# zyt334/AdaFace

Measured on AMD Instinct MI355X. Metric: 512x512 images/sec @ 50 DDIM steps, batch 8, higher is better.
Workload: dtype bf16

## Files before the change

### adaface_amd/csrc/af_conv_s8.hip

```cpp
#include "af_kernels.h"

#include <type_traits>

namespace cs8 {
typedef bf16 T;
typedef __attribute__((ext_vector_type(4))) unsigned u32x4;
constexpr int BM = 256, BN = 80, NI = 5, MI = 2, SPLITK = 4;
constexpr int HSLOTS = 448, HBUF = HSLOTS * 128, NHQ = HSLOTS / 8 / 8;
constexpr int WBYTES = BN * 128, WPIECES = BN / 8, D = 3, NS = 4;
constexpr int W_BASE = 2 * HBUF, LDS_BYTES = W_BASE + NS * WBYTES;
static_assert(LDS_BYTES <= 160 * 1024 && NHQ == 7, "LDS plan");

__device__ __forceinline__ void lds_dma16(__amdgpu_buffer_rsrc_t rs, char* lds_base, unsigned voffset, unsigned soffset) {
#if defined(__HIP_DEVICE_COMPILE__)
  __builtin_amdgcn_raw_ptr_buffer_load_lds(rs, (__attribute__((address_space(3))) void*)lds_base, 16, voffset, soffset, 0, 0);
#endif
}
__device__ __forceinline__ u32x4 lds_read128(unsigned addr) {
  u32x4 v;
  asm volatile("ds_read_b128 %0, %1" : "=v"(v) : "v"(addr) : "memory");
  return v;
}
template <int OFF> __device__ __forceinline__ u32x4 lds_read128o(unsigned addr) {
  u32x4 v;
  asm volatile("ds_read_b128 %0, %1 offset:%2" : "=v"(v) : "v"(addr), "n"(OFF) : "memory");
  return v;
}
template <int N> __device__ __forceinline__ void wait_vm() { asm volatile("s_waitcnt vmcnt(%0)" ::"n"(N) : "memory"); }
template <int N> __device__ __forceinline__ void wait_lgkm2(u32x4& a, u32x4& b) {
  asm volatile("s_waitcnt lgkmcnt(%2)" : "+v"(a), "+v"(b) : "n"(N) : "memory");
}
template <int N> __device__ __forceinline__ void wait_lgkm4(u32x4& a, u32x4& b, u32x4& c, u32x4& d) {
  asm volatile("s_waitcnt lgkmcnt(%4)" : "+v"(a), "+v"(b), "+v"(c), "+v"(d) : "n"(N) : "memory");
}
template <int I, int N, typename F> __device__ __forceinline__ void static_for(F&& f) {
  if constexpr (I < N) {
    f(std::integral_constant<int, I>{});
    static_for<I + 1, N>(f);
  }
}
__device__ __forceinline__ f32x4 mma(const u32x4& a, const u32x4& b, const f32x4& c) {
  return __builtin_amdgcn_mfma_f32_16x16x32_bf16(__builtin_bit_cast(bf16x8, a), __builtin_bit_cast(bf16x8, b), c, 0, 0, 0);
}

template <int SPLITK_T>
__global__ __launch_bounds__(512) void conv3x3_s8_kernel(const ConvGemmParams p) {
  extern __shared__ __attribute__((aligned(1024))) char smem[];
  const int tid = threadIdx.x, lane = tid & 63, wid = __builtin_amdgcn_readfirstlane(tid >> 6);
  const int l15 = lane & 15, g = lane >> 4;
  const int ntn = p.N / BN;
  const int tm = blockIdx.x / ntn, tn = blockIdx.x - tm * ntn;
  const int m0 = tm * BM, n0 = tn * BN, zk = blockIdx.z;
  const int nch = (p.Cin >> 6) / SPLITK_T, chunk0 = zk * nch;
  const __amdgpu_buffer_rsrc_t rs_x = __builtin_amdgcn_make_buffer_rsrc(const_cast<T*>(reinterpret_cast<const T*>(p.src)), 0, (int)0xFFFFFFF0u, 0x00020000);
  const __amdgpu_buffer_rsrc_t rs_w = __builtin_amdgcn_make_buffer_rsrc(const_cast<T*>(reinterpret_cast<const T*>(p.W)), 0, (int)0xFFFFFFF0u, 0x00020000);

  const int srow = lane >> 3;
  const unsigned dchunk = (unsigned)((lane & 7) ^ srow);
  const unsigned ldcb = (unsigned)p.ldc * 2u;
  const int wsh = p.wo_shift, Wo = 1 << wsh, HW = Wo + 2, hwsh = p.howo_shift;
  const int R = min(p.Ho, 256 >> wsh), HP1 = (R + 2) * HW, ipt = 256 / (R << wsh);
  const int img0 = m0 >> hwsh, y0 = (m0 & ((1 << hwsh) - 1)) >> wsh;
  unsigned h_off[NHQ];
#pragma unroll
  for (int q = 0; q < NHQ; ++q) {
    const int hp = (wid + 8 * q) * 8 + srow;
    const int img = hp / HP1, rem = hp - img * HP1, hy = rem / HW, hx = rem - hy * HW;
    const int iy = y0 + hy - 1, ix = hx - 1;
    const bool ok = img < ipt && (unsigned)iy < (unsigned)p.Ho && (unsigned)ix < (unsigned)Wo;
    h_off[q] = ok ? (unsigned)(((img0 + img) << hwsh) + (iy << wsh) + ix) * ldcb + dchunk * 16u : 0xFFFFFFFFu;
  }
  const int nwq = wid < WPIECES - 8 ? 2 : 1;
  unsigned w_off[2];
#pragma unroll
  for (int q = 0; q < 2; ++q) w_off[q] = (unsigned)((n0 + (wid + 8 * q) * 8 + srow) * p.ldw * 2) + dchunk * 16u;

  const int nsteps = nch * 9;
  auto stage_w = [&](int s, int slot) {
    const int c = s / 9, tap = s - 9 * c;
    const bool live = s < nsteps;
    const unsigned k0b = (unsigned)(tap * p.Cin + (chunk0 + c) * 64) * 2u;
    lds_dma16(rs_w, smem + W_BASE + slot * WBYTES + wid * 1024, live ? w_off[0] : 0xFFFFFFFFu, k0b);
    if (wid < WPIECES - 8) lds_dma16(rs_w, smem + W_BASE + slot * WBYTES + (wid + 8) * 1024, live ? w_off[1] : 0xFFFFFFFFu, k0b);
  };
  auto stage_h = [&](auto qc, int hbuf, int c) {
    constexpr int q = decltype(qc)::value;
    const bool live = c < nch;
    lds_dma16(rs_x, smem + hbuf * HBUF + (wid + 8 * q) * 1024, live ? h_off[q] : 0xFFFFFFFFu, (unsigned)(chunk0 + c) * 128u);
  };

  const unsigned lds0 = (unsigned)(__UINTPTR_TYPE__)((__attribute__((address_space(3))) char*)smem);
  const unsigned fch0 = (unsigned)(g ^ (lane & 7)) * 16u, fch1 = (unsigned)((g + 4) ^ (lane & 7)) * 16u;
  const unsigned w_base = (unsigned)(l15 * 128);
  int xhp[MI];
#pragma unroll
  for (int j = 0; j < MI; ++j) {
    const int t = wid * 32 + j * 16 + l15;
    const int part = t / (R << wsh), yl = (t >> wsh) - part * R;
    xhp[j] = part * HP1 + yl * HW + (t & (Wo - 1));
  }
  f32x4 acc[NI][MI];
#pragma unroll
  for (int i = 0; i < NI; ++i)
#pragma unroll
    for (int j = 0; j < MI; ++j) acc[i][j] = f32x4{0.f, 0.f, 0.f, 0.f};

  static_for<0, NHQ>([&](auto qc) { stage_h(qc, 0, 0); });
#pragma unroll
  for (int s = 0; s < D; ++s) stage_w(s, s);

  u32x4 xs[2][MI][2], wh[2][2][2];
#pragma unroll
  for (int j = 0; j < MI; ++j) xs[1][j][0] = xs[1][j][1] = u32x4{0u, 0u, 0u, 0u};
#pragma unroll
  for (int b2 = 0; b2 < 2; ++b2) wh[1][b2][0] = wh[1][b2][1] = u32x4{0u, 0u, 0u, 0u};
  int hb = 0, slot = 0;
  for (int c = 0; c < nch; ++c) {
    static_for<0, 9>([&](auto tc) {
      constexpr int tap = decltype(tc)::value;
      constexpr int cs = tap & 1, ps = cs ^ 1;
      constexpr int hyoung = tap == 0 ? 0 : (tap == 1 ? 1 : (tap == 2 ? 2 : (tap <= 7 ? 3 : 2)));
      if (nwq == 2) wait_vm<2 * (D - 1) + hyoung>(); else wait_vm<(D - 1) + hyoung>();
      __builtin_amdgcn_s_barrier();
      constexpr int ky = tap / 3, kx = tap - 3 * ky;
      const int tapoff = ky * HW + kx;
      unsigned xa[MI];
#pragma unroll
      for (int j = 0; j < MI; ++j) {
        const unsigned hp = (unsigned)(xhp[j] + tapoff);
        xa[j] = lds0 + (unsigned)(hb * HBUF) + (hp << 7) + ((((unsigned)g ^ hp) & 7u) << 4);
      }
      const unsigned wa0 = lds0 + (unsigned)(W_BASE + slot * WBYTES) + w_base + fch0;
      const unsigned wa1 = lds0 + (unsigned)(W_BASE + slot * WBYTES) + w_base + fch1;
      u32x4 wf[3][2];
#pragma unroll
      for (int j = 0; j < MI; ++j) {
        xs[cs][j][0] = lds_read128(xa[j]);
        xs[cs][j][1] = lds_read128(xa[j] ^ 64u);
      }
      wf[0][0] = lds_read128o<0 * 2048>(wa0); wf[0][1] = lds_read128o<0 * 2048>(wa1);
      wf[1][0] = lds_read128o<1 * 2048>(wa0); wf[1][1] = lds_read128o<1 * 2048>(wa1);
      wf[2][0] = lds_read128o<2 * 2048>(wa0); wf[2][1] = lds_read128o<2 * 2048>(wa1);
      __builtin_amdgcn_sched_barrier(0);
#pragma unroll
      for (int b2 = 0; b2 < 2; ++b2)
#pragma unroll
        for (int j = 0; j < MI; ++j) {
          acc[3 + b2][j] = mma(wh[ps][b2][0], xs[ps][j][0], acc[3 + b2][j]);
          acc[3 + b2][j] = mma(wh[ps][b2][1], xs[ps][j][1], acc[3 + b2][j]);
          asm volatile("" : "+v"(acc[3 + b2][j]));
        }
      __builtin_amdgcn_sched_barrier(0);
      wait_lgkm4<4>(xs[cs][0][0], xs[cs][0][1], xs[cs][1][0], xs[cs][1][1]);
      wait_lgkm2<4>(wf[0][0], wf[0][1]);
#pragma unroll
      for (int j = 0; j < MI; ++j) {
        acc[0][j] = mma(wf[0][0], xs[cs][j][0], acc[0][j]);
        acc[0][j] = mma(wf[0][1], xs[cs][j][1], acc[0][j]);
        asm volatile("" : "+v"(acc[0][j]));
      }
      wh[cs][0][0] = lds_read128o<3 * 2048>(wa0); wh[cs][0][1] = lds_read128o<3 * 2048>(wa1);
      __builtin_amdgcn_sched_barrier(0);
      wait_lgkm2<4>(wf[1][0], wf[1][1]);
#pragma unroll
      for (int j = 0; j < MI; ++j) {
        acc[1][j] = mma(wf[1][0], xs[cs][j][0], acc[1][j]);
        acc[1][j] = mma(wf[1][1], xs[cs][j][1], acc[1][j]);
        asm volatile("" : "+v"(acc[1][j]));
      }
      stage_w(c * 9 + tap + D, (slot + D) & (NS - 1));
      if constexpr (tap < NHQ) stage_h(std::integral_constant<int, tap>{}, hb ^ 1, c + 1);
      wh[cs][1][0] = lds_read128o<4 * 2048>(wa0); wh[cs][1][1] = lds_read128o<4 * 2048>(wa1);
      __builtin_amdgcn_sched_barrier(0);
      wait_lgkm2<4>(wf[2][0], wf[2][1]);
#pragma unroll
      for (int j = 0; j < MI; ++j) {
        acc[2][j] = mma(wf[2][0], xs[cs][j][0], acc[2][j]);
        acc[2][j] = mma(wf[2][1], xs[cs][j][1], acc[2][j]);
        asm volatile("" : "+v"(acc[2][j]));
      }
      __builtin_amdgcn_sched_barrier(0);
      asm volatile("s_waitcnt lgkmcnt(0)"
                   : "+v"(wh[cs][0][0]), "+v"(wh[cs][0][1]), "+v"(wh[cs][1][0]), "+v"(wh[cs][1][1])
                   :
                   : "memory");
      slot = (slot + 1) & (NS - 1);
    });
#pragma unroll
    for (int j = 0; j < MI; ++j) { xs[1][j][0] = xs[0][j][0]; xs[1][j][1] = xs[0][j][1]; }
#pragma unroll
    for (int b2 = 0; b2 < 2; ++b2) { wh[1][b2][0] = wh[0][b2][0]; wh[1][b2][1] = wh[0][b2][1]; }
    hb ^= 1;
  }
#pragma unroll
  for (int b2 = 0; b2 < 2; ++b2)
#pragma unroll
    for (int j = 0; j < MI; ++j) {
      acc[3 + b2][j] = mma(wh[1][b2][0], xs[1][j][0], acc[3 + b2][j]);
      acc[3 + b2][j] = mma(wh[1][b2][1], xs[1][j][1], acc[3 + b2][j]);
    }
  wait_vm<0>();

  if constexpr (SPLITK_T > 1) {
    float* slab = reinterpret_cast<float*>(p.ws) + (long)zk * p.M * p.N;
#pragma unroll
    for (int j = 0; j < MI; ++j) {
      const int m = m0 + wid * 32 + j * 16 + l15;
#pragma unroll
      for (int i = 0; i < NI; ++i) *reinterpret_cast<f32x4*>(slab + (long)m * p.N + n0 + i * 16 + 4 * g) = acc[i][j];
    }
  } else {
    __builtin_amdgcn_s_barrier();
    constexpr int OPITCH = BN * 2 + 16, OCH = BN / 8, NST = 32 * OCH / 64;
    char* otile = smem + wid * (32 * OPITCH);
    const T* res = reinterpret_cast<const T*>(p.residual);
    const T* rowb = reinterpret_cast<const T*>(p.rowbias);
    const int cl = 4 * g;
    float4 bvec[NI];
    Quad<T> bq[NI];
#pragma unroll
    for (int i = 0; i < NI; ++i) {
      bvec[i] = p.bias ? *reinterpret_cast<const float4*>(p.bias + n0 + i * 16 + cl) : float4{0.f, 0.f, 0.f, 0.f};
      if (rowb) bq[i].load(rowb + (long)(m0 >> p.howo_shift) * p.ldrb + n0 + i * 16 + cl);
    }
#pragma unroll
    for (int j = 0; j < MI; ++j) {
      const int m = m0 + wid * 32 + j * 16 + l15;
      Quad<T> rq[NI];
      if (res) {
#pragma unroll
        for (int i = 0; i < NI; ++i) rq[i].load(res + (long)m * p.ldr + n0 + i * 16 + cl);
      }
#pragma unroll
      for (int i = 0; i < NI; ++i) {
        const float* bp = reinterpret_cast<const float*>(&bvec[i]);
        Quad<T> o;
#pragma unroll
        for (int e = 0; e < 4; ++e) {
          float v = acc[i][j][e] + bp[e];
          if (rowb) v += to_f32<T>(bq[i].e[e]);
          if (res) v += to_f32<T>(rq[i].e[e]);
          o.e[e] = from_f32<T>(v);
        }
        o.store(reinterpret_cast<T*>(otile + (j * 16 + l15) * OPITCH) + i * 16 + cl);
      }
    }
    const __amdgpu_buffer_rsrc_t rs_o = __builtin_amdgcn_make_buffer_rsrc(reinterpret_cast<T*>(p.out), 0, (int)0xFFFFFFF0u, 0x00020000);
    u32x4 chunk[NST];
    unsigned orow[NST];
#pragma unroll
    for (int i = 0; i < NST; ++i) {
      const unsigned c = (unsigned)(lane + 64 * i), row = c / OCH, ch = c - row * OCH;
      orow[i] = (unsigned)(m0 + wid * 32 + (int)row) * (unsigned)(p.ldo * 2) + ch * 16u;
      chunk[i] = *reinterpret_cast<const u32x4*>(otile + row * OPITCH + ch * 16);
    }
    __builtin_amdgcn_sched_barrier(0);
#pragma unroll
    for (int i = 0; i < NST; ++i) __builtin_amdgcn_raw_buffer_store_b128(chunk[i], rs_o, orow[i], n0 * 2, 0);
    __builtin_amdgcn_sched_barrier(0);
  }
}
}

int af_conv_s8_slices(const ConvGemmParams& p, int batch) {
  auto pow2 = [](int v) { return v > 0 && (v & (v - 1)) == 0; };
  if (batch != 1 || p.fp8 || p.ks != 3 || p.stride != 1 || p.pad != 1 || p.up != 0 || p.Hi != p.Ho || p.Wi != p.Wo ||
      p.Hs != p.Ho || p.Ws != p.Wo || !pow2(p.Wo) || !pow2(p.Ho) || p.Wo < 8 || p.Wo > 64 || p.M <= 0 || p.M % cs8::BM != 0 || p.N % cs8::BN != 0 ||
      p.K != 9 * p.Cin || p.ldc < p.Cin || p.ldc % 8 != 0 || p.epilogue != AF_EPI_NONE || p.ln_stats || p.ln_stats_out || p.gn_ab || p.phase4 ||
      p.src_batch_stride != (long)p.Ho * p.Wo * p.ldc)
    return 0;
  const int R = p.Ho < 256 / p.Wo ? p.Ho : 256 / p.Wo;
  if (256 % (R * p.Wo) != 0 || (256 / (R * p.Wo)) * (R + 2) * (p.Wo + 2) > cs8::HSLOTS || (p.Ho * p.Wo > 256 && p.Ho % R != 0)) return 0;
  if (p.Wo == 8 && p.Ho == 8) return p.Cin % (64 * cs8::SPLITK) == 0 ? cs8::SPLITK : 0;
  return (p.Cin % 64 == 0 && p.ldo % 8 == 0 && (!p.residual || p.ldr % 4 == 0) && (!p.rowbias || p.ldrb % 4 == 0) && ((__UINTPTR_TYPE__)p.out & 15) == 0 &&
          (long)(p.M / cs8::BM) * (p.N / cs8::BN) >= 128) ? 1 : 0;
}
int af_launch_conv_s8(const ConvGemmParams& p, hipStream_t stream) {
  static unsigned long long attr_done4 = 0, attr_done1 = 0;
  const int sl = af_conv_s8_slices(p, 1);
  if (sl == 0 || p.splitk != sl || (sl > 1 && !p.ws) || p.wo_shift < 3 || p.howo_shift < p.wo_shift) {
    af_set_error_msg("conv_s8: shape / slice count %d not taken by the small-map kernel", p.splitk);
    return -1;
  }
  const dim3 grid((p.M / cs8::BM) * (p.N / cs8::BN), 1, sl);
  if (sl > 1) {
    if (int rc = af_ensure_dynamic_lds(attr_done4, reinterpret_cast<const void*>(&cs8::conv3x3_s8_kernel<cs8::SPLITK>), cs8::LDS_BYTES)) return rc;
    hipLaunchKernelGGL(cs8::conv3x3_s8_kernel<cs8::SPLITK>, grid, dim3(512), cs8::LDS_BYTES, stream, p);
  } else {
    if (int rc = af_ensure_dynamic_lds(attr_done1, reinterpret_cast<const void*>(&cs8::conv3x3_s8_kernel<1>), cs8::LDS_BYTES)) return rc;
    hipLaunchKernelGGL(cs8::conv3x3_s8_kernel<1>, grid, dim3(512), cs8::LDS_BYTES, stream, p);
  }
  HIP_CHECK_RET(hipGetLastError());
  return 0;
}
```

### adaface_amd/csrc/af_conv_gemm_pp_body.h

```cpp
  static_assert(SCHED == 0 || SCHED == 2, "schedules: 0 phased, 2 merged");
  constexpr bool MG = SCHED == 2;
  constexpr bool FT = GATHER && MG;
  static_assert(MG || !FP8, "fp8 operands exist on the merged schedule only");
  using C = PpCfg<BN>;
  typedef bf16 T;
  static_assert(!FP8 || LNMODE == 0, "fp8 operands: plain epilogue only");
  constexpr unsigned XE = FP8 ? 1u : 2u;
  constexpr int NI = C::NI, MI = C::MI, SLOT = C::SLOT, XBYTES = C::XBYTES;
  constexpr int XP0 = MG ? C::XP / 2 : C::XP0;
  constexpr int NX0 = XP0 / 4, NX1 = (C::XP - XP0) / 4;
  constexpr int WP0 = MG ? (C::WP / 8) * 4 : 0;
  constexpr int NW0 = WP0 / 4, NW1 = (C::WP - WP0) / 4;
  constexpr int NP0 = NX0 + NW0, NP1 = NX1 + NW1, NPMAX = NP0 > NP1 ? NP0 : NP1;
  constexpr int NXM = NX0 > NX1 ? NX0 : NX1, NWM = NW0 > NW1 ? NW0 : NW1;
  static_assert(XP0 % 4 == 0 && WP0 % 4 == 0 && NW1 >= 1, "piece split");
  extern __shared__ __attribute__((aligned(1024))) char smem[];

  const int tid = threadIdx.x, lane = tid & 63, wid = __builtin_amdgcn_readfirstlane(tid >> 6);
  const int g = wid >> 2, wq = wid & 3;
  const int ntm = (p.M + 255) / 256, ntn = p.N / BN;
  int tm, tn;
  tile_coords(blockIdx.x, gridDim.x, ntm, ntn, p.group_m, tm, tn);
  const int m0 = tm * 256, n0 = tn * BN;
  const int zk = blockIdx.z;
// ... 166 lines not shown

  const unsigned lds0 = (unsigned)(__UINTPTR_TYPE__)((__attribute__((address_space(3))) char*)smem);
  const unsigned fch0 = (unsigned)((lane >> 4) ^ (lane & 7)) * 16u;
  const unsigned fch1 = (unsigned)(((lane >> 4) + 4) ^ (lane & 7)) * 16u;
  const unsigned x_base = (unsigned)((wq * 64 + (lane & 15)) * 128);
  const unsigned w_base = (unsigned)(XBYTES + (g * C::HN + (lane & 15)) * 128);

  f32x4 acc[NI][MI];
#pragma unroll
  for (int i = 0; i < NI; ++i)
#pragma unroll
    for (int j = 0; j < MI; ++j) acc[i][j] = f32x4{0.f, 0.f, 0.f, 0.f};
  pp_u32x4 xf[MI][2], wf[NI][2];
#pragma unroll
  for (int i = 0; i < NI; ++i) wf[i][1] = pp_u32x4{0u, 0u, 0u, 0u};
#pragma unroll
  for (int j = 0; j < MI; ++j) xf[j][1] = pp_u32x4{0u, 0u, 0u, 0u};

  auto half = [&](int slot_off, auto rc, auto mc) {
    constexpr int ur = decltype(rc)::value, um = decltype(mc)::value;
    const unsigned b = lds0 + (unsigned)slot_off + (ur ? fch1 : fch0);
    pp_static_for<0, NI * MI>([&](auto nc) {
      constexpr int n = decltype(nc)::value;
      constexpr int i = n / MI, j = n % MI;
      if constexpr (n < NI) wf[n][ur] = pp_lds_read128<n * 2048>(b + w_base);
      else if constexpr (n < NI + MI) xf[n - NI][ur] = pp_lds_read128<(n - NI) * 2048>(b + x_base);
      acc[i][j] = __builtin_amdgcn_mfma_f32_16x16x32_bf16(__builtin_bit_cast(bf16x8, wf[i][um]),
                                                          __builtin_bit_cast(bf16x8, xf[j][um]), acc[i][j], 0, 0, 0);
      if constexpr (n < NI + MI) __builtin_amdgcn_sched_barrier(0);
    });
  };
  std::integral_constant<int, 0> U0;
  std::integral_constant<int, 1> U1;

  const int cl = 4 * (lane >> 4);
  float4 bias_r[NI];
  auto load_bias = [&]() {
#pragma unroll
    for (int i = 0; i < NI; ++i) {
      bias_r[i] = float4{0.f, 0.f, 0.f, 0.f};
      if (p.bias && p.splitk <= 1) bias_r[i] = *reinterpret_cast<const float4*>(p.bias + n0 + g * C::HN + i * 16 + cl);
    }
  };
  if constexpr (!MG) load_bias();

  float4 ln_cs[LNMODE == 1 ? NI : 1];
  float ln_mu[LNMODE == 1 ? MI : 1], ln_rs[LNMODE == 1 ? MI : 1];
  if constexpr (LNMODE == 1) {
#pragma unroll
    for (int i = 0; i < NI; ++i) ln_cs[i] = *reinterpret_cast<const float4*>(p.ln_colsum + n0 + g * C::HN + i * 16 + cl);
#pragma unroll
    for (int j = 0; j < MI; ++j) {
      const int m = m0 + wq * 64 + j * 16 + (lane & 15);
      float2 st = float2{0.f, 0.f};
      if (m < p.M) st = *reinterpret_cast<const float2*>(p.ln_stats + (long)m * 2);
      ln_mu[j] = st.x;
      ln_rs[j] = st.y;
    }
  }

  pp_u32x4 w8[MG ? NI : 1][2], xa8[MG ? MI : 1][2], xb8[MG ? MI : 1][2];
  int wsc8[FP8 ? NI : 1];
  int xsc8 = p.x_scale_e8;
  if constexpr (MG && !FP8) {
#pragma unroll
    for (int i = 0; i < NI; ++i) w8[i][0] = w8[i][1] = pp_u32x4{0u, 0u, 0u, 0u};
#pragma unroll
    for (int j = 0; j < MI; ++j) xa8[j][0] = xa8[j][1] = xb8[j][0] = xb8[j][1] = pp_u32x4{0u, 0u, 0u, 0u};
  }
  if constexpr (FP8) {
    asm volatile("" : "+v"(xsc8));
#pragma unroll
    for (int i = 0; i < NI; ++i) {
      w8[i][0] = w8[i][1] = pp_u32x4{0u, 0u, 0u, 0u};
      wsc8[i] = (int)p.w_scale[n0 + g * C::HN + i * 16 + (lane & 15)];
    }
#pragma unroll
    for (int j = 0; j < MI; ++j) xa8[j][0] = xa8[j][1] = xb8[j][0] = xb8[j][1] = pp_u32x4{0u, 0u, 0u, 0u};
  }
  auto mfma8 = [&](f32x4& c, const pp_u32x4 (&wv)[2], const pp_u32x4 (&xv)[2], int wscale) {
    if constexpr (!FP8) {
      c = __builtin_amdgcn_mfma_f32_16x16x32_bf16(__builtin_bit_cast(bf16x8, wv[0]), __builtin_bit_cast(bf16x8, xv[0]), c, 0, 0, 0);
      c = __builtin_amdgcn_mfma_f32_16x16x32_bf16(__builtin_bit_cast(bf16x8, wv[1]), __builtin_bit_cast(bf16x8, xv[1]), c, 0, 0, 0);
      asm volatile("" : "+v"(c));
      return;
    }
    const pp_i32x8 a = __builtin_shufflevector(__builtin_bit_cast(pp_i32x4, wv[0]), __builtin_bit_cast(pp_i32x4, wv[1]), 0, 1, 2, 3, 4, 5, 6, 7);
    const pp_i32x8 b = __builtin_shufflevector(__builtin_bit_cast(pp_i32x4, xv[0]), __builtin_bit_cast(pp_i32x4, xv[1]), 0, 1, 2, 3, 4, 5, 6, 7);
    c = __builtin_amdgcn_mfma_scale_f32_16x16x128_f8f6f4(a, b, c, 0, 0, 0, wscale, 0, xsc8);
    asm volatile("" : "+v"(c));
  };
  auto wait_block = [&](auto nc, pp_u32x4 (&blk)[2]) {
    constexpr int n = decltype(nc)::value;
    asm volatile("s_waitcnt lgkmcnt(%2)" : "+v"(blk[0]), "+v"(blk[1]) : "n"(n) : "memory");
  };
#ifdef AF_LAB_ABLATE
  const int lab = p.ablate >> 4;
#else
  constexpr int lab = 0;
#endif
  auto cphase8 = [&](int slot_off, pp_u32x4 (&xc)[MG ? MI : 1][2], pp_u32x4 (&xp)[MG ? MI : 1][2], int stage_off,
                     const StageCtx& sc) {
    if constexpr (MG) {
      constexpr int NB = NI + MI;
      char* sbase = smem + stage_off;
      const unsigned b0 = lds0 + (unsigned)slot_off + fch0, b1 = lds0 + (unsigned)slot_off + fch1;
      auto rd_block = [&](auto bc) {
        constexpr int bi = decltype(bc)::value;
        if (lab & 2) return;
        if constexpr (bi == 0) {
          w8[0][0] = pp_lds_read128<0>(b0 + w_base);
          w8[0][1] = pp_lds_read128<0>(b1 + w_base);
        } else if constexpr (bi <= MI) {
          xc[bi - 1][0] = pp_lds_read128<(bi - 1) * 2048>(b0 + x_base);
          xc[bi - 1][1] = pp_lds_read128<(bi - 1) * 2048>(b1 + x_base);
        } else {
          w8[bi - MI][0] = pp_lds_read128<(bi - MI) * 2048>(b0 + w_base);
          w8[bi - MI][1] = pp_lds_read128<(bi - MI) * 2048>(b1 + w_base);
        }
      };
      rd_block(std::integral_constant<int, 0>{});
      rd_block(std::integral_constant<int, 1>{});
      __builtin_amdgcn_sched_barrier(0);
      pp_static_for<0, MI * NI>([&](auto mc) {
        constexpr int m = decltype(mc)::value;
        if constexpr (m < MI) {
          if (!(lab & 4)) mfma8(acc[NI - 1][m], w8[NI - 1], xp[m], wsc8[FP8 ? NI - 1 : 0]);
        } else {
          constexpr int i = (m - MI) / MI, j = (m - MI) % MI;
          constexpr int issued = (2 + m) < NB ? (2 + m) : NB;
          constexpr int need = i == 0 ? 1 + j : (j == 0 ? MI + i : -1);
          if constexpr (need >= 0) {
            std::integral_constant<int, 2 * (issued - need - 1)> cnt;
            if constexpr (i == 0) wait_block(cnt, xc[j]); else wait_block(cnt, w8[i]);
            if constexpr (i == 0 && j == 0) wait_block(cnt, w8[0]);
          }
          if (!(lab & 4)) mfma8(acc[i][j], w8[i], xc[j], wsc8[FP8 ? i : 0]);
        }
        if constexpr (2 + m < NB) rd_block(std::integral_constant<int, 2 + m>{});
        if constexpr (m >= MI && (m - MI) / 2 < NPMAX) {
          if (!(lab & 1) && g == ((m - MI) & 1)) stage_piece(std::integral_constant<int, (m - MI) / 2>{}, sbase, sc);
        }
        __builtin_amdgcn_sched_barrier(0);
      });
      static_assert(MI + 2 * (NPMAX - 1) + 1 < MI * NI, "merged schedule: a staging slot behind an MFMA for every piece");
      pp_wait_lgkm0();
    }
  };

  int rd = 0, w0 = SLOT, w1 = 2 * SLOT;
  if constexpr (MG) {
    stage(0);
    stage(SLOT);
    auto tile = [&](auto& xc, auto& xp) {
      if (g == 0) pp_wait_vm<NP0>(); else pp_wait_vm<NP1>();
      __builtin_amdgcn_s_barrier();
      const StageCtx sc = stage_begin(kw);
      cphase8(rd, xc, xp, w1, sc);
      kw = kw_next(kw);
      const int tmp = rd; rd = w0; w0 = w1; w1 = tmp;
    };
    for (int t = 0; t + 1 < KT; t += 2) {
      tile(xa8, xb8);
      tile(xb8, xa8);
    }
    if (KT & 1) tile(xa8, xb8);
    pp_wait_vm<0>();
    if (KT & 1) {
#pragma unroll
      for (int j = 0; j < MI; ++j) mfma8(acc[NI - 1][j], w8[NI - 1], xa8[j], wsc8[FP8 ? NI - 1 : 0]);
    } else {
#pragma unroll
      for (int j = 0; j < MI; ++j) mfma8(acc[NI - 1][j], w8[NI - 1], xb8[j], wsc8[FP8 ? NI - 1 : 0]);
    }
    __builtin_amdgcn_s_barrier();
  } else {
    auto wait_keep1 = [&]() { if (g == 0) pp_wait_vm<NP0>(); else pp_wait_vm<NP1>(); };
    stage(0);
    if (g == 1) {
      if (KT > 1) { stage(SLOT); wait_keep1(); } else pp_wait_vm<0>();
    }
    __builtin_amdgcn_s_barrier();
    if (g == 1) __builtin_amdgcn_s_barrier();
    auto dphase = [&](int t) {
      if (g == 0) {
        if (t + 1 < KT) { stage(w0); wait_keep1(); } else pp_wait_vm<0>();
      } else {
        if (t + 2 < KT) stage(w1);
      }
      __builtin_amdgcn_s_barrier();
    };
    auto cend = [&](int t) {
      if (g == 1) { if (t + 2 < KT) wait_keep1(); else pp_wait_vm<0>(); }
      __builtin_amdgcn_s_barrier();
      const int tmp = rd; rd = w0; w0 = w1; w1 = tmp;
    };
    for (int t = 0; t < KT; ++t) {
      dphase(t);
      __builtin_amdgcn_s_setprio(1);
      half(rd, U0, U1);
      pp_wait_lgkm0();
      half(rd, U1, U0);
      pp_wait_lgkm0();
      __builtin_amdgcn_s_setprio(0);
      cend(t);
    }
#pragma unroll
    for (int i = 0; i < NI; ++i)
#pragma unroll
      for (int j = 0; j < MI; ++j)
        acc[i][j] = __builtin_amdgcn_mfma_f32_16x16x32_bf16(__builtin_bit_cast(bf16x8, wf[i][1]),
                                                            __builtin_bit_cast(bf16x8, xf[j][1]), acc[i][j], 0, 0, 0);
    if (g == 0) __builtin_amdgcn_s_barrier();
  }
  if constexpr (MG) load_bias();
```

Before: 10.95.

## Rework small-map 3x3 conv to 4 waves with 64-row warp tiles and deeper pipelining

Result: no change. 10.99 (median of 6 runs) (+0.4%).

```diff
diff --git a/adaface_amd/csrc/af_conv_s8.hip b/adaface_amd/csrc/af_conv_s8.hip
--- a/adaface_amd/csrc/af_conv_s8.hip
+++ b/adaface_amd/csrc/af_conv_s8.hip
@@ -5,11 +5,13 @@
 namespace cs8 {
 typedef bf16 T;
 typedef __attribute__((ext_vector_type(4))) unsigned u32x4;
-constexpr int BM = 256, BN = 80, NI = 5, MI = 2, SPLITK = 4;
-constexpr int HSLOTS = 448, HBUF = HSLOTS * 128, NHQ = HSLOTS / 8 / 8;
+constexpr int BM = 256, BN = 80, NI = 5, SPLITK = 4;
+constexpr int MI = 4, NHQ = 448 / 8 / 4;
+constexpr int MI8 = 2;
+constexpr int HSLOTS = 448, HBUF = HSLOTS * 128, NHQ8 = HSLOTS / 8 / 8;
 constexpr int WBYTES = BN * 128, WPIECES = BN / 8, D = 3, NS = 4;
 constexpr int W_BASE = 2 * HBUF, LDS_BYTES = W_BASE + NS * WBYTES;
-static_assert(LDS_BYTES <= 160 * 1024 && NHQ == 7, "LDS plan");
+static_assert(LDS_BYTES <= 160 * 1024 && NHQ8 == 7 && NHQ == 14 && NS == 4, "LDS plan");
 
 __device__ __forceinline__ void lds_dma16(__amdgpu_buffer_rsrc_t rs, char* lds_base, unsigned voffset, unsigned soffset) {
 #if defined(__HIP_DEVICE_COMPILE__)
@@ -43,8 +45,16 @@
   return __builtin_amdgcn_mfma_f32_16x16x32_bf16(__builtin_bit_cast(bf16x8, a), __builtin_bit_cast(bf16x8, b), c, 0, 0, 0);
 }
 
+template <int N> __device__ __forceinline__ void wait_lgkm_xw(u32x4 (&x)[MI][2], u32x4 (&w)[3][2]) {
+  asm volatile("s_waitcnt lgkmcnt(%14)"
+               : "+v"(x[0][0]), "+v"(x[0][1]), "+v"(x[1][0]), "+v"(x[1][1]), "+v"(x[2][0]), "+v"(x[2][1]), "+v"(x[3][0]), "+v"(x[3][1]),
+                 "+v"(w[0][0]), "+v"(w[0][1]), "+v"(w[1][0]), "+v"(w[1][1]), "+v"(w[2][0]), "+v"(w[2][1])
+               : "n"(N)
+               : "memory");
+}
+
 template <int SPLITK_T>
-__global__ __launch_bounds__(512) void conv3x3_s8_kernel(const ConvGemmParams p) {
+__global__ __launch_bounds__(256) void conv3x3_s8_kernel(const ConvGemmParams p) {
   extern __shared__ __attribute__((aligned(1024))) char smem[];
   const int tid = threadIdx.x, lane = tid & 63, wid = __builtin_amdgcn_readfirstlane(tid >> 6);
   const int l15 = lane & 15, g = lane >> 4;
@@ -61,9 +71,245 @@
   const int wsh = p.wo_shift, Wo = 1 << wsh, HW = Wo + 2, hwsh = p.howo_shift;
   const int R = min(p.Ho, 256 >> wsh), HP1 = (R + 2) * HW, ipt = 256 / (R << wsh);
   const int img0 = m0 >> hwsh, y0 = (m0 & ((1 << hwsh) - 1)) >> wsh;
+  const unsigned mg_hp1 = (1u << 18) / (unsigned)HP1 + 1u, mg_hw = (1u << 18) / (unsigned)HW + 1u;
   unsigned h_off[NHQ];
 #pragma unroll
   for (int q = 0; q < NHQ; ++q) {
+    const int hp = (wid + 4 * q) * 8 + srow;
+    const int img = (int)(((unsigned)hp * mg_hp1) >> 18), rem = hp - img * HP1, hy = (int)(((unsigned)rem * mg_hw) >> 18), hx = rem - hy * HW;
+    const int iy = y0 + hy - 1, ix = hx - 1;
+    const bool ok = img < ipt && (unsigned)iy < (unsigned)p.Ho && (unsigned)ix < (unsigned)Wo;
+    h_off[q] = ok ? (unsigned)(((img0 + img) << hwsh) + (iy << wsh) + ix) * ldcb + dchunk * 16u : 0xFFFFFFFFu;
+  }
+  const int nw = wid < WPIECES - 8 ? 3 : 2;
+  unsigned w_off[3];
+#pragma unroll
+  for (int q = 0; q < 3; ++q) w_off[q] = (unsigned)((n0 + (wid + 4 * q) * 8 + srow) * p.ldw * 2) + dchunk * 16u;
+
+  auto stage_w = [&](auto qc, int c, int tap, int slot) {
+    constexpr int q = decltype(qc)::value;
+    const unsigned k0b = (unsigned)(tap * p.Cin + (chunk0 + c) * 64) * 2u;
+    lds_dma16(rs_w, smem + W_BASE + slot * WBYTES + (wid + 4 * q) * 1024, c < nch ? w_off[q] : 0xFFFFFFFFu, k0b);
+  };
+  auto stage_h = [&](auto qc, int hbuf, int c) {
+    constexpr int q = decltype(qc)::value;
+    lds_dma16(rs_x, smem + hbuf * HBUF + (wid + 4 * q) * 1024, c < nch ? h_off[q] : 0xFFFFFFFFu, (unsigned)(chunk0 + c) * 128u);
+  };
+
+  const unsigned lds0 = (unsigned)(__UINTPTR_TYPE__)((__attribute__((address_space(3))) char*)smem);
+  const unsigned fch0 = (unsigned)(g ^ (lane & 7)) * 16u, fch1 = (unsigned)((g + 4) ^ (lane & 7)) * 16u;
+  const unsigned w_base = (unsigned)(l15 * 128);
+  int xhp[MI];
+#pragma unroll
+  for (int j = 0; j < MI; ++j) {
+    const int t = wid * 64 + j * 16 + l15;
+    const int part = t >> min(hwsh, 8), yl = (t >> wsh) - part * R;
+    xhp[j] = part * HP1 + yl * HW + (t & (Wo - 1));
+  }
+  f32x4 acc[NI][MI];
+#pragma unroll
+  for (int i = 0; i < NI; ++i)
+#pragma unroll
+    for (int j = 0; j < MI; ++j) acc[i][j] = f32x4{0.f, 0.f, 0.f, 0.f};
+
+  u32x4 xs[2][MI][2], wf[2][3][2], wr[2][2];
+  auto xaddr = [&](int j, int hbuf, int tapoff) {
+    const unsigned hp = (unsigned)(xhp[j] + tapoff);
+    return lds0 + (unsigned)(hbuf * HBUF) + (hp << 7) + ((((unsigned)g ^ hp) & 7u) << 4);
+  };
+
+  static_for<0, NHQ>([&](auto qc) { stage_h(qc, 0, 0); });
+#pragma unroll
+  for (int s = 0; s < NS; ++s) {
+    stage_w(std::integral_constant<int, 0>{}, 0, s, s);
+    stage_w(std::integral_constant<int, 1>{}, 0, s, s);
+    if (nw == 3) stage_w(std::integral_constant<int, 2>{}, 0, s, s);
+  }
+  if (nw == 3) wait_vm<3 * 3>(); else wait_vm<3 * 2>();
+  __builtin_amdgcn_s_barrier();
+#pragma unroll
+  for (int j = 0; j < MI; ++j) {
+    const unsigned xa = xaddr(j, 0, 0);
+    xs[0][j][0] = lds_read128(xa);
+    xs[0][j][1] = lds_read128(xa ^ 64u);
+  }
+  wf[0][0][0] = lds_read128o<0 * 2048>(lds0 + (unsigned)W_BASE + w_base + fch0); wf[0][0][1] = lds_read128o<0 * 2048>(lds0 + (unsigned)W_BASE + w_base + fch1);
+  wf[0][1][0] = lds_read128o<1 * 2048>(lds0 + (unsigned)W_BASE + w_base + fch0); wf[0][1][1] = lds_read128o<1 * 2048>(lds0 + (unsigned)W_BASE + w_base + fch1);
+  wf[0][2][0] = lds_read128o<2 * 2048>(lds0 + (unsigned)W_BASE + w_base + fch0); wf[0][2][1] = lds_read128o<2 * 2048>(lds0 + (unsigned)W_BASE + w_base + fch1);
+
+  auto blk = [&](auto ic, u32x4 (&x)[MI][2], u32x4& wa, u32x4& wb, auto&& f) {
+    constexpr int i = decltype(ic)::value;
+    acc[i][0] = mma(wa, x[0][0], acc[i][0]);
+    acc[i][1] = mma(wa, x[1][0], acc[i][1]);
+    f(std::integral_constant<int, 0>{});
+    __builtin_amdgcn_sched_barrier(0);
+    acc[i][2] = mma(wa, x[2][0], acc[i][2]);
+    acc[i][3] = mma(wa, x[3][0], acc[i][3]);
+    f(std::integral_constant<int, 1>{});
+    __builtin_amdgcn_sched_barrier(0);
+    acc[i][0] = mma(wb, x[0][1], acc[i][0]);
+    acc[i][1] = mma(wb, x[1][1], acc[i][1]);
+    f(std::integral_constant<int, 2>{});
+    __builtin_amdgcn_sched_barrier(0);
+    acc[i][2] = mma(wb, x[2][1], acc[i][2]);
+    acc[i][3] = mma(wb, x[3][1], acc[i][3]);
+    f(std::integral_constant<int, 3>{});
+    asm volatile("" : "+v"(acc[i][0]), "+v"(acc[i][1]), "+v"(acc[i][2]), "+v"(acc[i][3]));
+    __builtin_amdgcn_sched_barrier(0);
+  };
+  int hb = 0, slot = 0;
+  auto chunk_body = [&](auto parc, int c) {
+    constexpr int PAR = decltype(parc)::value;
+    static_for<0, 9>([&](auto tc) {
+      constexpr int tap = decltype(tc)::value;
+      constexpr int cs = (tap + PAR) & 1, ns = cs ^ 1;
+      constexpr int tap1 = (tap + 1) % 9, ky1 = tap1 / 3, kx1 = tap1 - 3 * ky1;
+      const unsigned wsl = lds0 + (unsigned)(W_BASE + slot * WBYTES) + w_base;
+      const unsigned wa0 = wsl + fch0, wa1 = wsl + fch1;
+      wait_lgkm_xw<0>(xs[cs], wf[cs]);
+      blk(std::integral_constant<int, 0>{}, xs[cs], wf[cs][0][0], wf[cs][0][1], [&](auto kc) {
+        constexpr int k = decltype(kc)::value;
+        if constexpr (k < 2) {
+          wr[k][0] = lds_read128o<(k + 3) * 2048>(wa0);
+          wr[k][1] = lds_read128o<(k + 3) * 2048>(wa1);
+        }
+      });
+      blk(std::integral_constant<int, 1>{}, xs[cs], wf[cs][1][0], wf[cs][1][1], [](auto) {});
+      wait_lgkm4<0>(wr[0][0], wr[0][1], wr[1][0], wr[1][1]);
+      constexpr int hyoung = (tap == 0 || tap == 8) ? 0 : (tap == 1 ? 2 : 4);
+      if (nw == 3) wait_vm<2 * 3 + hyoung>(); else wait_vm<2 * 2 + hyoung>();
+      __builtin_amdgcn_s_barrier();
+      const int hb1 = tap == 8 ? hb ^ 1 : hb;
+      const int tapoff1 = ky1 * HW + kx1;
+      unsigned xa[MI];
+#pragma unroll
+      for (int j = 0; j < MI; ++j) xa[j] = xaddr(j, hb1, tapoff1);
+      const unsigned wsl1 = lds0 + (unsigned)(W_BASE + ((slot + 1) & (NS - 1)) * WBYTES) + w_base;
+      const unsigned wn0 = wsl1 + fch0, wn1 = wsl1 + fch1;
+      __builtin_amdgcn_sched_barrier(0);
+      blk(std::integral_constant<int, 2>{}, xs[cs], wf[cs][2][0], wf[cs][2][1], [&](auto kc) {
+        constexpr int k = decltype(kc)::value;
+        xs[ns][k][0] = lds_read128(xa[k]);
+        xs[ns][k][1] = lds_read128(xa[k] ^ 64u);
+      });
+      blk(std::integral_constant<int, 3>{}, xs[cs], wr[0][0], wr[0][1], [&](auto kc) {
+        constexpr int k = decltype(kc)::value;
+        if constexpr (k < 3) {
+          wf[ns][k][0] = lds_read128o<k * 2048>(wn0);
+          wf[ns][k][1] = lds_read128o<k * 2048>(wn1);
+        }
+      });
+      constexpr int tap4 = (tap + NS) % 9;
+      const int c4 = tap + NS < 9 ? c : c + 1;
+      blk(std::integral_constant<int, 4>{}, xs[cs], wr[1][0], wr[1][1], [&](auto kc) {
+        constexpr int k = decltype(kc)::value;
+        if constexpr (k == 0) {
+          if constexpr (2 * tap + 1 < NHQ) {
+            stage_h(std::integral_constant<int, 2 * tap>{}, hb ^ 1, c + 1);
+            stage_h(std::integral_constant<int, 2 * tap + 1>{}, hb ^ 1, c + 1);
+          }
+        } else if constexpr (k == 1) {
+          stage_w(std::integral_constant<int, 0>{}, c4, tap4, slot);
+        } else if constexpr (k == 2) {
+          stage_w(std::integral_constant<int, 1>{}, c4, tap4, slot);
+        } else {
+          if (nw == 3) stage_w(std::integral_constant<int, 2>{}, c4, tap4, slot);
+        }
+      });
+      slot = (slot + 1) & (NS - 1);
+    });
+    hb ^= 1;
+  };
+  for (int c = 0; c < nch; c += 2) {
+    chunk_body(std::integral_constant<int, 0>{}, c);
+    if (c + 1 < nch) chunk_body(std::integral_constant<int, 1>{}, c + 1);
+  }
+  wait_lgkm_xw<0>(xs[0], wf[0]);
+  wait_lgkm_xw<0>(xs[1], wf[1]);
+  wait_vm<0>();
+
+  if constexpr (SPLITK_T > 1) {
+    float* slab = reinterpret_cast<float*>(p.ws) + (long)zk * p.M * p.N;
+#pragma unroll
+    for (int j = 0; j < MI; ++j) {
+      const int m = m0 + wid * 64 + j * 16 + l15;
+#pragma unroll
+      for (int i = 0; i < NI; ++i) *reinterpret_cast<f32x4*>(slab + (long)m * p.N + n0 + i * 16 + 4 * g) = acc[i][j];
+    }
+  } else {
+    __builtin_amdgcn_s_barrier();
+    constexpr int OPITCH = BN * 2 + 16, OCH = BN / 8, NST = 64 * OCH / 64;
+    static_assert(4 * 64 * OPITCH <= 2 * HBUF, "transposition tiles");
+    char* otile = smem + wid * (64 * OPITCH);
+    const T* res = reinterpret_cast<const T*>(p.residual);
+    const T* rowb = reinterpret_cast<const T*>(p.rowbias);
+    const int cl = 4 * g;
+    float4 bvec[NI];
+    Quad<T> bq[NI];
+#pragma unroll
+    for (int i = 0; i < NI; ++i) {
+      bvec[i] = p.bias ? *reinterpret_cast<const float4*>(p.bias + n0 + i * 16 + cl) : float4{0.f, 0.f, 0.f, 0.f};
+      if (rowb) bq[i].load(rowb + (long)(m0 >> p.howo_shift) * p.ldrb + n0 + i * 16 + cl);
+    }
+#pragma unroll
+    for (int j = 0; j < MI; ++j) {
+      const int m = m0 + wid * 64 + j * 16 + l15;
+      Quad<T> rq[NI];
+      if (res) {
+#pragma unroll
+        for (int i = 0; i < NI; ++i) rq[i].load(res + (long)m * p.ldr + n0 + i * 16 + cl);
+      }
+#pragma unroll
+      for (int i = 0; i < NI; ++i) {
+        const float* bp = reinterpret_cast<const float*>(&bvec[i]);
+        Quad<T> o;
+#pragma unroll
+        for (int e = 0; e < 4; ++e) {
+          float v = acc[i][j][e] + bp[e];
+          if (rowb) v += to_f32<T>(bq[i].e[e]);
+          if (res) v += to_f32<T>(rq[i].e[e]);
+          o.e[e] = from_f32<T>(v);
+        }
+        o.store(reinterpret_cast<T*>(otile + (j * 16 + l15) * OPITCH) + i * 16 + cl);
+      }
+    }
+    const __amdgpu_buffer_rsrc_t rs_o = __builtin_amdgcn_make_buffer_rsrc(reinterpret_cast<T*>(p.out), 0, (int)0xFFFFFFF0u, 0x00020000);
+    u32x4 chunk[NST];
+    unsigned orow[NST];
+#pragma unroll
+    for (int i = 0; i < NST; ++i) {
+      const unsigned c = (unsigned)(lane + 64 * i), row = c / OCH, ch = c - row * OCH;
+      orow[i] = (unsigned)(m0 + wid * 64 + (int)row) * (unsigned)(p.ldo * 2) + ch * 16u;
+      chunk[i] = *reinterpret_cast<const u32x4*>(otile + row * OPITCH + ch * 16);
+    }
+    __builtin_amdgcn_sched_barrier(0);
+#pragma unroll
+    for (int i = 0; i < NST; ++i) __builtin_amdgcn_raw_buffer_store_b128(chunk[i], rs_o, orow[i], n0 * 2, 0);
+    __builtin_amdgcn_sched_barrier(0);
+  }
+}
+
+template <int SPLITK_T>
+__global__ __launch_bounds__(512) void conv3x3_s8_w8_kernel(const ConvGemmParams p) {
+  extern __shared__ __attribute__((aligned(1024))) char smem[];
+  const int tid = threadIdx.x, lane = tid & 63, wid = __builtin_amdgcn_readfirstlane(tid >> 6);
+  const int l15 = lane & 15, g = lane >> 4;
+  const int ntn = p.N / BN;
+  const int tm = blockIdx.x / ntn, tn = blockIdx.x - tm * ntn;
+  const int m0 = tm * BM, n0 = tn * BN, zk = blockIdx.z;
+  const int nch = (p.Cin >> 6) / SPLITK_T, chunk0 = zk * nch;
+  const __amdgpu_buffer_rsrc_t rs_x = __builtin_amdgcn_make_buffer_rsrc(const_cast<T*>(reinterpret_cast<const T*>(p.src)), 0, (int)0xFFFFFFF0u, 0x00020000);
+  const __amdgpu_buffer_rsrc_t rs_w = __builtin_amdgcn_make_buffer_rsrc(const_cast<T*>(reinterpret_cast<const T*>(p.W)), 0, (int)0xFFFFFFF0u, 0x00020000);
+
+  const int srow = lane >> 3;
+  const unsigned dchunk = (unsigned)((lane & 7) ^ srow);
+  const unsigned ldcb = (unsigned)p.ldc * 2u;
+  const int wsh = p.wo_shift, Wo = 1 << wsh, HW = Wo + 2, hwsh = p.howo_shift;
+  const int R = min(p.Ho, 256 >> wsh), HP1 = (R + 2) * HW, ipt = 256 / (R << wsh);
+  const int img0 = m0 >> hwsh, y0 = (m0 & ((1 << hwsh) - 1)) >> wsh;
+  unsigned h_off[NHQ8];
+#pragma unroll
+  for (int q = 0; q < NHQ8; ++q) {
     const int hp = (wid + 8 * q) * 8 + srow;
     const int img = hp / HP1, rem = hp - img * HP1, hy = rem / HW, hx = rem - hy * HW;
     const int iy = y0 + hy - 1, ix = hx - 1;
@@ -92,26 +338,26 @@
   const unsigned lds0 = (unsigned)(__UINTPTR_TYPE__)((__attribute__((address_space(3))) char*)smem);
   const unsigned fch0 = (unsigned)(g ^ (lane & 7)) * 16u, fch1 = (unsigned)((g + 4) ^ (lane & 7)) * 16u;
   const unsigned w_base = (unsigned)(l15 * 128);
-  int xhp[MI];
-#pragma unroll
-  for (int j = 0; j < MI; ++j) {
+  int xhp[MI8];
+#pragma unroll
+  for (int j = 0; j < MI8; ++j) {
     const int t = wid * 32 + j * 16 + l15;
     const int part = t / (R << wsh), yl = (t >> wsh) - part * R;
     xhp[j] = part * HP1 + yl * HW + (t & (Wo - 1));
   }
-  f32x4 acc[NI][MI];
+  f32x4 acc[NI][MI8];
 #pragma unroll
   for (int i = 0; i < NI; ++i)
 #pragma unroll
-    for (int j = 0; j < MI; ++j) acc[i][j] = f32x4{0.f, 0.f, 0.f, 0.f};
-
-  static_for<0, NHQ>([&](auto qc) { stage_h(qc, 0, 0); });
+    for (int j = 0; j < MI8; ++j) acc[i][j] = f32x4{0.f, 0.f, 0.f, 0.f};
+
+  static_for<0, NHQ8>([&](auto qc) { stage_h(qc, 0, 0); });
 #pragma unroll
   for (int s = 0; s < D; ++s) stage_w(s, s);
 
-  u32x4 xs[2][MI][2], wh[2][2][2];
-#pragma unroll
-  for (int j = 0; j < MI; ++j) xs[1][j][0] = xs[1][j][1] = u32x4{0u, 0u, 0u, 0u};
+  u32x4 xs[2][MI8][2], wh[2][2][2];
+#pragma unroll
+  for (int j = 0; j < MI8; ++j) xs[1][j][0] = xs[1][j][1] = u32x4{0u, 0u, 0u, 0u};
 #pragma unroll
   for (int b2 = 0; b2 < 2; ++b2) wh[1][b2][0] = wh[1][b2][1] = u32x4{0u, 0u, 0u, 0u};
   int hb = 0, slot = 0;
@@ -124,9 +370,9 @@
       __builtin_amdgcn_s_barrier();
       constexpr int ky = tap / 3, kx = tap - 3 * ky;
       const int tapoff = ky * HW + kx;
-      unsigned xa[MI];
-#pragma unroll
-      for (int j = 0; j < MI; ++j) {
+      unsigned xa[MI8];
+#pragma unroll
+      for (int j = 0; j < MI8; ++j) {
         const unsigned hp = (unsigned)(xhp[j] + tapoff);
         xa[j] = lds0 + (unsigned)(hb * HBUF) + (hp << 7) + ((((unsigned)g ^ hp) & 7u) << 4);
       }
@@ -134,7 +380,7 @@
       const unsigned wa1 = lds0 + (unsigned)(W_BASE + slot * WBYTES) + w_base + fch1;
       u32x4 wf[3][2];
 #pragma unroll
-      for (int j = 0; j < MI; ++j) {
+      for (int j = 0; j < MI8; ++j) {
         xs[cs][j][0] = lds_read128(xa[j]);
         xs[cs][j][1] = lds_read128(xa[j] ^ 64u);
       }
@@ -145,7 +391,7 @@
 #pragma unroll
       for (int b2 = 0; b2 < 2; ++b2)
 #pragma unroll
-        for (int j = 0; j < MI; ++j) {
+        for (int j = 0; j < MI8; ++j) {
           acc[3 + b2][j] = mma(wh[ps][b2][0], xs[ps][j][0], acc[3 + b2][j]);
           acc[3 + b2][j] = mma(wh[ps][b2][1], xs[ps][j][1], acc[3 + b2][j]);
           asm volatile("" : "+v"(acc[3 + b2][j]));
@@ -154,7 +400,7 @@
       wait_lgkm4<4>(xs[cs][0][0], xs[cs][0][1], xs[cs][1][0], xs[cs][1][1]);
       wait_lgkm2<4>(wf[0][0], wf[0][1]);
 #pragma unroll
-      for (int j = 0; j < MI; ++j) {
+      for (int j = 0; j < MI8; ++j) {
         acc[0][j] = mma(wf[0][0], xs[cs][j][0], acc[0][j]);
         acc[0][j] = mma(wf[0][1], xs[cs][j][1], acc[0][j]);
         asm volatile("" : "+v"(acc[0][j]));
@@ -163,18 +409,18 @@
       __builtin_amdgcn_sched_barrier(0);
       wait_lgkm2<4>(wf[1][0], wf[1][1]);
 #pragma unroll
-      for (int j = 0; j < MI; ++j) {
+      for (int j = 0; j < MI8; ++j) {
         acc[1][j] = mma(wf[1][0], xs[cs][j][0], acc[1][j]);
         acc[1][j] = mma(wf[1][1], xs[cs][j][1], acc[1][j]);
         asm volatile("" : "+v"(acc[1][j]));
       }
       stage_w(c * 9 + tap + D, (slot + D) & (NS - 1));
-      if constexpr (tap < NHQ) stage_h(std::integral_constant<int, tap>{}, hb ^ 1, c + 1);
+      if constexpr (tap < NHQ8) stage_h(std::integral_constant<int, tap>{}, hb ^ 1, c + 1);
       wh[cs][1][0] = lds_read128o<4 * 2048>(wa0); wh[cs][1][1] = lds_read128o<4 * 2048>(wa1);
       __builtin_amdgcn_sched_barrier(0);
       wait_lgkm2<4>(wf[2][0], wf[2][1]);
 #pragma unroll
-      for (int j = 0; j < MI; ++j) {
+      for (int j = 0; j < MI8; ++j) {
         acc[2][j] = mma(wf[2][0], xs[cs][j][0], acc[2][j]);
         acc[2][j] = mma(wf[2][1], xs[cs][j][1], acc[2][j]);
         asm volatile("" : "+v"(acc[2][j]));
@@ -187,7 +433,7 @@
       slot = (slot + 1) & (NS - 1);
     });
 #pragma unroll
-    for (int j = 0; j < MI; ++j) { xs[1][j][0] = xs[0][j][0]; xs[1][j][1] = xs[0][j][1]; }
+    for (int j = 0; j < MI8; ++j) { xs[1][j][0] = xs[0][j][0]; xs[1][j][1] = xs[0][j][1]; }
 #pragma unroll
     for (int b2 = 0; b2 < 2; ++b2) { wh[1][b2][0] = wh[0][b2][0]; wh[1][b2][1] = wh[0][b2][1]; }
     hb ^= 1;
@@ -195,7 +441,7 @@
 #pragma unroll
   for (int b2 = 0; b2 < 2; ++b2)
 #pragma unroll
-    for (int j = 0; j < MI; ++j) {
+    for (int j = 0; j < MI8; ++j) {
       acc[3 + b2][j] = mma(wh[1][b2][0], xs[1][j][0], acc[3 + b2][j]);
       acc[3 + b2][j] = mma(wh[1][b2][1], xs[1][j][1], acc[3 + b2][j]);
     }
@@ -204,7 +450,7 @@
   if constexpr (SPLITK_T > 1) {
     float* slab = reinterpret_cast<float*>(p.ws) + (long)zk * p.M * p.N;
 #pragma unroll
-    for (int j = 0; j < MI; ++j) {
+    for (int j = 0; j < MI8; ++j) {
       const int m = m0 + wid * 32 + j * 16 + l15;
 #pragma unroll
       for (int i = 0; i < NI; ++i) *reinterpret_cast<f32x4*>(slab + (long)m * p.N + n0 + i * 16 + 4 * g) = acc[i][j];
@@ -224,7 +470,7 @@
       if (rowb) bq[i].load(rowb + (long)(m0 >> p.howo_shift) * p.ldrb + n0 + i * 16 + cl);
     }
 #pragma unroll
-    for (int j = 0; j < MI; ++j) {
+    for (int j = 0; j < MI8; ++j) {
       const int m = m0 + wid * 32 + j * 16 + l15;
       Quad<T> rq[NI];
       if (res) {
@@ -272,23 +518,30 @@
   const int R = p.Ho < 256 / p.Wo ? p.Ho : 256 / p.Wo;
   if (256 % (R * p.Wo) != 0 || (256 / (R * p.Wo)) * (R + 2) * (p.Wo + 2) > cs8::HSLOTS || (p.Ho * p.Wo > 256 && p.Ho % R != 0)) return 0;
   if (p.Wo == 8 && p.Ho == 8) return p.Cin % (64 * cs8::SPLITK) == 0 ? cs8::SPLITK : 0;
-  return (p.Cin % 64 == 0 && p.ldo % 8 == 0 && (!p.residual || p.ldr % 4 == 0) && (!p.rowbias || p.ldrb % 4 == 0) && ((__UINTPTR_TYPE__)p.out & 15) == 0 &&
+  return (p.alpha == 1.0f && p.Cin % 64 == 0 && p.ldo % 8 == 0 && (!p.residual || p.ldr % 4 == 0) && (!p.rowbias || p.ldrb % 4 == 0) && ((__UINTPTR_TYPE__)p.out & 15) == 0 &&
           (long)(p.M / cs8::BM) * (p.N / cs8::BN) >= 128) ? 1 : 0;
 }
 int af_launch_conv_s8(const ConvGemmParams& p, hipStream_t stream) {
-  static unsigned long long attr_done4 = 0, attr_done1 = 0;
+  static unsigned long long attr_done4 = 0, attr_done1 = 0, attr_done4_w8 = 0, attr_done1_w8 = 0;
   const int sl = af_conv_s8_slices(p, 1);
   if (sl == 0 || p.splitk != sl || (sl > 1 && !p.ws) || p.wo_shift < 3 || p.howo_shift < p.wo_shift) {
     af_set_error_msg("conv_s8: shape / slice count %d not taken by the small-map kernel", p.splitk);
     return -1;
   }
   const dim3 grid((p.M / cs8::BM) * (p.N / cs8::BN), 1, sl);
-  if (sl > 1) {
+  const bool w8 = (g_af_knobs.conv_halo8 & 8) != 0;
+  if (sl > 1 && w8) {
+    if (int rc = af_ensure_dynamic_lds(attr_done4_w8, reinterpret_cast<const void*>(&cs8::conv3x3_s8_w8_kernel<cs8::SPLITK>), cs8::LDS_BYTES)) return rc;
+    hipLaunchKernelGGL(cs8::conv3x3_s8_w8_kernel<cs8::SPLITK>, grid, dim3(512), cs8::LDS_BYTES, stream, p);
+  } else if (sl > 1) {
     if (int rc = af_ensure_dynamic_lds(attr_done4, reinterpret_cast<const void*>(&cs8::conv3x3_s8_kernel<cs8::SPLITK>), cs8::LDS_BYTES)) return rc;
-    hipLaunchKernelGGL(cs8::conv3x3_s8_kernel<cs8::SPLITK>, grid, dim3(512), cs8::LDS_BYTES, stream, p);
+    hipLaunchKernelGGL(cs8::conv3x3_s8_kernel<cs8::SPLITK>, grid, dim3(256), cs8::LDS_BYTES, stream, p);
+  } else if (w8) {
+    if (int rc = af_ensure_dynamic_lds(attr_done1_w8, reinterpret_cast<const void*>(&cs8::conv3x3_s8_w8_kernel<1>), cs8::LDS_BYTES)) return rc;
+    hipLaunchKernelGGL(cs8::conv3x3_s8_w8_kernel<1>, grid, dim3(512), cs8::LDS_BYTES, stream, p);
   } else {
     if (int rc = af_ensure_dynamic_lds(attr_done1, reinterpret_cast<const void*>(&cs8::conv3x3_s8_kernel<1>), cs8::LDS_BYTES)) return rc;
-    hipLaunchKernelGGL(cs8::conv3x3_s8_kernel<1>, grid, dim3(512), cs8::LDS_BYTES, stream, p);
+    hipLaunchKernelGGL(cs8::conv3x3_s8_kernel<1>, grid, dim3(256), cs8::LDS_BYTES, stream, p);
   }
   HIP_CHECK_RET(hipGetLastError());
   return 0;
```

## Add compile-time unrolled 3x3 tap walk for bf16 gather conv K-loop

Applied to the files above, without the earlier changes.

Measured after the change: 10.55 before, 10.58 after, median of 6. Within noise of the previous version (+0.3%).

```diff
diff --git a/adaface_amd/csrc/af_conv_gemm_pp_body.h b/adaface_amd/csrc/af_conv_gemm_pp_body.h
--- a/adaface_amd/csrc/af_conv_gemm_pp_body.h
+++ b/adaface_amd/csrc/af_conv_gemm_pp_body.h
@@ -342,6 +342,112 @@
   if constexpr (MG) {
     stage(0);
     stage(SLOT);
+    constexpr bool KW = !FP8 && GATHER && BN == 128;
+    bool kwalk = false;
+    T* const xsrc = const_cast<T*>(reinterpret_cast<const T*>(p.src));
+    T* const wsrc = const_cast<T*>(reinterpret_cast<const T*>(p.W));
+    const unsigned wrd0 = lds0 + w_base + fch0, wrd1 = lds0 + w_base + fch1;
+    const unsigned xrd0 = lds0 + x_base + fch0, xrd1 = lds0 + x_base + fch1;
+    auto kstep = [&](auto gc, auto sc, auto&& piece) {
+      constexpr int G = decltype(gc)::value, S = decltype(sc)::value;
+      constexpr int NB = NI + MI, NPG = G == 0 ? NP0 : NP1;
+      constexpr unsigned RD = (unsigned)(S * SLOT);
+      pp_wait_vm<NPG>();
+      __builtin_amdgcn_s_barrier();
+      const unsigned w0a = wrd0 + RD, w1a = wrd1 + RD, x0a = xrd0 + RD, x1a = xrd1 + RD;
+      pp_u32x4 xc[MI][2];
+      auto rd_block = [&](auto bc) {
+        constexpr int bi = decltype(bc)::value;
+        if (lab & 2) return;
+        if constexpr (bi == 0) {
+          w8[0][0] = pp_lds_read128<0>(w0a);
+          w8[0][1] = pp_lds_read128<0>(w1a);
+        } else if constexpr (bi <= MI) {
+          xc[bi - 1][0] = pp_lds_read128<(bi - 1) * 2048>(x0a);
+          xc[bi - 1][1] = pp_lds_read128<(bi - 1) * 2048>(x1a);
+        } else {
+          w8[bi - MI][0] = pp_lds_read128<(bi - MI) * 2048>(w0a);
+          w8[bi - MI][1] = pp_lds_read128<(bi - MI) * 2048>(w1a);
+        }
+      };
+      rd_block(std::integral_constant<int, 0>{});
+      rd_block(std::integral_constant<int, 1>{});
+      __builtin_amdgcn_sched_barrier(0);
+      pp_static_for<0, MI * NI>([&](auto mc) {
+        constexpr int m = decltype(mc)::value;
+        if constexpr (m < MI) {
+          if (!(lab & 4)) mfma8(acc[NI - 1][m], w8[NI - 1], xa8[m], 0);
+        } else {
+          constexpr int i = (m - MI) / MI, j = (m - MI) % MI;
+          constexpr int issued = (2 + m) < NB ? (2 + m) : NB;
+          constexpr int need = i == 0 ? 1 + j : (j == 0 ? MI + i : -1);
+          if constexpr (need >= 0) {
+            std::integral_constant<int, 2 * (issued - need - 1)> cnt;
+            if constexpr (i == 0) wait_block(cnt, xc[j]); else wait_block(cnt, w8[i]);
+            if constexpr (i == 0 && j == 0) wait_block(cnt, w8[0]);
+          }
+          if (!(lab & 4)) mfma8(acc[i][j], w8[i], xc[j], 0);
+        }
+        if constexpr (2 + m < NB) rd_block(std::integral_constant<int, 2 + m>{});
+        if constexpr (m >= MI && (m - MI) / 2 < NPG && ((m - MI) & 1) == G) {
+          if (!(lab & 1)) piece(std::integral_constant<int, (m - MI) / 2>{});
+        }
+        __builtin_amdgcn_sched_barrier(0);
+      });
+      pp_wait_lgkm0();
+#pragma unroll
+      for (int j = 0; j < MI; ++j) xa8[j][0] = xc[j][0], xa8[j][1] = xc[j][1];
+    };
+   if constexpr (KW) {
+    kwalk = p.ks == 3 && !p.phase4 && kt_begin % 9 == 0 && KT % 9 == 0;
+    if (kwalk) {
+      const unsigned cin2 = (unsigned)p.Cin * 2u;
+      const unsigned rowb = (unsigned)p.Ws * ldcb;
+      const int nch = KT / 9;
+#pragma unroll
+      for (int q = 0; q < NXM; ++q) {
+        x_yx[q] = ~x_yx[q];
+#ifdef AF_LAB_ABLATE
+        if (p.ablate & 0x100) x_yx[q] |= ~1;
+#endif
+      }
+      auto gstep = [&](auto gc, auto tc, const __amdgpu_buffer_rsrc_t& rs_xn, const __amdgpu_buffer_rsrc_t& rs_wn, unsigned kc) {
+        constexpr int G = decltype(gc)::value, TAP = decltype(tc)::value;
+        constexpr int NXG = G == 0 ? NX0 : NX1;
+        constexpr int XQ0 = G == 0 ? 0 : XP0, WQ0 = G == 0 ? 0 : WP0;
+        constexpr int TS = (TAP + 2) % 9, KYS = TS / 3, KXS = TS % 3;
+        constexpr bool NEXT = TAP + 2 >= 9;
+        constexpr unsigned ST = (unsigned)((TS % 3) * SLOT);
+        const unsigned delta = (unsigned)KYS * rowb + (unsigned)KXS * ldcb;
+        const unsigned kcs = NEXT ? kc + 128u : kc;
+        const unsigned kws = (unsigned)TS * cin2 + kcs;
+        char* const xdst = smem + ST + (XQ0 + wq) * 1024;
+        char* const wdst = smem + ST + XBYTES + (WQ0 + wq) * 1024;
+        kstep(gc, std::integral_constant<int, TAP % 3>{}, [&](auto qc) {
+          constexpr int q = decltype(qc)::value;
+          if constexpr (q < NXG) {
+            asm volatile("" : "+v"(x_yx[q]));
+            const unsigned a = (x_off[q] + delta) | (unsigned)((int)((unsigned)x_yx[q] << (31 - TS)) >> 31);
+            lds_dma16(NEXT ? rs_xn : rs_x, xdst + 4 * q * 1024, a, kcs);
+          } else {
+            lds_dma16(NEXT ? rs_wn : rs_w, wdst + 4 * (q - NXG) * 1024, w_off[q - NXG], kws);
+          }
+        });
+      };
+      auto gloop = [&](auto gc) {
+        unsigned kc = (unsigned)(kt_begin / 9) * 128u;
+        for (int c = 0; c < nch; ++c) {
+          const int nrec = c + 1 < nch ? (int)0xFFFFFFF0u : 0;
+          const __amdgpu_buffer_rsrc_t rs_xn = __builtin_amdgcn_make_buffer_rsrc(xsrc, 0, nrec, 0x00020000);
+          const __amdgpu_buffer_rsrc_t rs_wn = __builtin_amdgcn_make_buffer_rsrc(wsrc, 0, nrec, 0x00020000);
+          pp_static_for<0, 9>([&](auto tc) { gstep(gc, tc, rs_xn, rs_wn, kc); });
+          kc += 128u;
+        }
+      };
+      if (g == 0) gloop(std::integral_constant<int, 0>{}); else gloop(std::integral_constant<int, 1>{});
+    }
+   }
+   if (!kwalk) {
     auto tile = [&](auto& xc, auto& xp) {
       if (g == 0) pp_wait_vm<NP0>(); else pp_wait_vm<NP1>();
       __builtin_amdgcn_s_barrier();
@@ -355,8 +461,9 @@
       tile(xb8, xa8);
     }
     if (KT & 1) tile(xa8, xb8);
+   }
     pp_wait_vm<0>();
-    if (KT & 1) {
+    if (kwalk || (KT & 1)) {
 #pragma unroll
       for (int j = 0; j < MI; ++j) mfma8(acc[NI - 1][j], w8[NI - 1], xa8[j], wsc8[FP8 ? NI - 1 : 0]);
     } else {
```
